# akio-tomiya/LatticeQCD.jl

Hardware: AMD Instinct MI355X
Metric: CG iters/sec (D^+D) & Dslash GFLOP/s, 32^3x64 SU(3) Wilson fp64 (higher is better)
Workload: dtype f64; 1 GPU; configs[3]: 32x32x32x64 Wilson D^+D CG (fixed-length window), fp64; dslash_variant=1, xcd_remap=2, xcd_nsub=16, xcd_ysplit=4, cg_fused=3, gauge_recon=12, gauge_recon_active=1, comm_backend=none, comm_requested=auto

## Files before the change

### latticeqcd.jl_amd/csrc/capi.hip

```cpp
#include "lqcd_internal.h"

#include <cstdio>
#include <cstdlib>
#include <cstring>
#include <mutex>

namespace lqcd {

static thread_local std::string g_err;
static std::mutex g_live_mu;
static std::vector<const lqcd_ctx_s*> g_live;
bool ctx_is_live(const lqcd_ctx_s* c) {
    std::lock_guard<std::mutex> lk(g_live_mu);
    for (const lqcd_ctx_s* p : g_live)
        if (p == c) return true;
    return false;
}
static void ctx_set_live(const lqcd_ctx_s* c, bool live) {
    std::lock_guard<std::mutex> lk(g_live_mu);
    for (size_t i = 0; i < g_live.size(); i++)
        if (g_live[i] == c) { g_live.erase(g_live.begin() + i); break; }
    if (live) g_live.push_back(c);
}
bool ctx_park_gauge(lqcd_gauge_s* g) {
    std::lock_guard<std::mutex> lk(g_live_mu);
    lqcd_ctx_s* c = g->ctx;
    bool live = false;
    for (const lqcd_ctx_s* p : g_live) live = live || p == c;
    if (!live || !c->tun.lazy_links || std::this_thread::get_id() == c->home_thread) return false;
    c->parked_gauges.push_back(g);
    return true;
}
int ctx_drain_parked(lqcd_ctx_s* c) {
    std::vector<lqcd_gauge_s*> mine;
    {
        std::lock_guard<std::mutex> lk(g_live_mu);
        mine.swap(c->parked_gauges);
    }
    for (lqcd_gauge_s* g : mine) (void)gauge_destroy_now(g);
    return LQCD_OK;
}
void set_error(const std::string& msg) { g_err = msg; }
int hip_fail(hipError_t e, const char* what, const char* file, int line) {
    g_err = std::string("HIP error: ") + hipGetErrorString(e) + " in " + what + " (" + file + ":" + std::to_string(line) + ")";
    (void)hipGetLastError();
    return LQCD_ERR_HIP;
}
int nccl_fail(ncclResult_t e, const char* what, const char* file, int line) {
    g_err = std::string("RCCL error: ") + ncclGetErrorString(e) + " in " + what + " (" + file + ":" + std::to_string(line) + ")";
    return LQCD_ERR_COMM;
}

lqcd_spinor_s* scratch_get(lqcd_ctx_s* c, int kind, int subset) {
    if (std::this_thread::get_id() == c->home_thread && !c->parked_gauges.empty()) (void)ctx_drain_parked(c);
    const int want_sub = subset == LQCD_FULL ? LQCD_FULL : LQCD_EVEN;
    for (lqcd_spinor_s* s : c->scratch)
        if (!s->in_use && s->kind == kind && (s->subset == LQCD_FULL) == (want_sub == LQCD_FULL)) {
            s->in_use = true;
            s->subset = subset;
            return s;
        }
    lqcd_spinor_s* s = nullptr;
    if (lqcd_spinor_create(c, &s, kind, subset) != LQCD_OK) return nullptr;
    s->in_use = true;
    c->scratch.push_back(s);
    return s;
}
void scratch_put(lqcd_spinor_s* s) {
    if (s) s->in_use = false;
}

int plaquette_local_sum(lqcd_gauge_s* g, const double2* const ghost[4], double* sum);
int gauge_pack_face(lqcd_gauge_s* g, int mu, double2* dst);

static int decompose(const int gL[4], const int pe[4], int rank, int L[4], int origin[4], int coord[4], int nf[4], int nb[4]) {
    int nranks = 1;
    for (int mu = 0; mu < 4; mu++) {
        ARGCHK(pe[mu] >= 1 && gL[mu] >= 2, "decompose: bad PE grid or lattice extent");
        ARGCHK(gL[mu] % pe[mu] == 0, "decompose: global extent not divisible by the PE grid");
        L[mu] = gL[mu] / pe[mu];
        ARGCHK(L[mu] % 2 == 0, "decompose: local extents must be even (checkerboard layout)");
        nranks *= pe[mu];
    }
    ARGCHK(rank >= 0 && rank < nranks, "decompose: rank outside the PE grid");
    int q = rank;
    for (int mu = 0; mu < 4; mu++) { coord[mu] = q % pe[mu]; q /= pe[mu]; origin[mu] = coord[mu] * L[mu]; }
    for (int mu = 0; mu < 4; mu++) {
        int cf[4] = {coord[0], coord[1], coord[2], coord[3]}, cb[4] = {coord[0], coord[1], coord[2], coord[3]};
        cf[mu] = (coord[mu] + 1) % pe[mu];
        cb[mu] = (coord[mu] + pe[mu] - 1) % pe[mu];
        nf[mu] = cf[0] + pe[0] * (cf[1] + pe[1] * (cf[2] + pe[2] * cf[3]));
        nb[mu] = cb[0] + pe[0] * (cb[1] + pe[1] * (cb[2] + pe[2] * cb[3]));
    }
    return LQCD_OK;
// ... 213 lines not shown
    if (!strcmp(key, "mixed_xfuse")) return &c->tun.mixed_xfuse;
    if (!strcmp(key, "mixed_defer_x")) return &c->tun.mixed_defer_x;
    if (!strcmp(key, "pair32_active")) return &c->tun.pair32_active;
    if (!strcmp(key, "stag_both")) return &c->tun.stag_both;
    if (!strcmp(key, "clover_fused")) return &c->tun.clover_fused;
    if (!strcmp(key, "clover_transport")) return &c->tun.clover_transport;
    if (!strcmp(key, "halo_stream_mode")) return &c->tun.halo_stream_mode;
    if (!strcmp(key, "cg_skip_done")) return &c->tun.cg_skip_done;
    if (!strcmp(key, "cg_small")) return &c->tun.cg_small;
    if (!strcmp(key, "cg_tgauge")) return &c->tun.cg_tgauge;
    if (!strcmp(key, "tgauge_active")) return &c->tun.tgauge_active;
    if (!strcmp(key, "cg_sweep_alt")) return &c->tun.cg_sweep_alt;
    if (!strcmp(key, "cg_sweep_alt_active")) return &c->tun.cg_sweep_alt_active;
    if (!strcmp(key, "dslash_sweep")) return &c->tun.dslash_sweep;
    if (!strcmp(key, "sweep_rev_active")) return &c->tun.sweep_rev_active;
    if (!strcmp(key, "dslash_xshare")) return &c->tun.dslash_xshare;
    if (!strcmp(key, "xshare_active")) return &c->tun.xshare_active;
    if (!strcmp(key, "dslash_yshare")) return &c->tun.dslash_yshare;
    if (!strcmp(key, "yshare_active")) return &c->tun.yshare_active;
    if (!strcmp(key, "nt_centre")) return &c->tun.nt_centre;
    if (!strcmp(key, "cg_persist")) return &c->tun.cg_persist;
    if (!strcmp(key, "md_remap")) return &c->tun.md_remap;
    if (!strcmp(key, "staple_recon")) return &c->tun.staple_recon;
    if (!strcmp(key, "staple_tile")) return &c->tun.staple_tile;
    if (!strcmp(key, "md_reunitarize")) return &c->tun.md_reunitarize;
    if (!strcmp(key, "nt_blas")) return &c->tun.nt_blas;
    if (!strcmp(key, "cg_fold_scalars")) return &c->tun.cg_fold_scalars;
    if (!strcmp(key, "halo_fuse")) return &c->tun.halo_fuse;
    if (!strcmp(key, "halo_fold")) return &c->tun.halo_fold;
    if (!strcmp(key, "halo_fold_active")) return &c->tun.halo_fold_active;
    if (!strcmp(key, "cg_defer_x")) return &c->tun.cg_defer_x;
    if (!strcmp(key, "cg_rring")) return &c->tun.cg_rring;
    if (!strcmp(key, "cg_rring_active")) return &c->tun.cg_rring_active;
    if (!strcmp(key, "staggered_parity_solve")) return &c->tun.staggered_parity_solve;
    if (!strcmp(key, "halo_tuned_us0")) return &c->tun.halo_tuned_us[0];
    if (!strcmp(key, "halo_tuned_us1")) return &c->tun.halo_tuned_us[1];
    if (!strcmp(key, "halo_tuned_us2")) return &c->tun.halo_tuned_us[2];
    if (!strcmp(key, "halo_tuned_us3")) return &c->tun.halo_tuned_us[3];
    if (!strcmp(key, "halo_tuned_us4")) return &c->tun.halo_tuned_us[4];
    if (!strcmp(key, "halo_inject_us")) return &c->tun.halo_inject_us;
    if (!strcmp(key, "halo_merge")) return &c->tun.halo_merge;
    if (!strcmp(key, "recon_active")) return &c->tun.recon_active;
    if (!strcmp(key, "variants_built")) return &c->tun.variants_built;
    if (!strcmp(key, "lds_pad_kb")) return &c->tun.lds_pad_kb;
    if (!strcmp(key, "xcd_nsub")) return &c->tun.xcd_nsub;
    if (!strcmp(key, "xcd_ysplit")) return &c->tun.xcd_ysplit;
#ifdef LQCD_ABLATE
    if (!strcmp(key, "dbg")) return &c->tun.dbg;
#endif
    if (!strcmp(key, "persist_per_cu")) return &c->tun.persist_per_cu;
    if (!strcmp(key, "dslash_pipe")) return &c->tun.dslash_pipe;
    if (!strcmp(key, "pipe_per_cu")) return &c->tun.pipe_per_cu;
    if (!strcmp(key, "pipe_grid")) return &c->tun.pipe_grid;
    if (!strcmp(key, "pipe_chunks_per_wg")) return &c->tun.pipe_chunks_per_wg;
    if (!strcmp(key, "pipe_min_chunks")) return &c->tun.pipe_min_chunks;
    if (!strcmp(key, "lazy_links")) return &c->tun.lazy_links;
    if (!strcmp(key, "lazy_merge")) return &c->tun.lazy_merge;
    if (!strcmp(key, "dw_batched")) return &c->tun.dw_batched;
    if (!strcmp(key, "dw_fused_cg")) return &c->tun.dw_fused_cg;
    if (!strcmp(key, "bicg_fused")) return &c->tun.bicg_fused;
    if (!strcmp(key, "gauge_delta")) return &c->tun.gauge_delta;
    if (!strcmp(key, "dslash_s18")) return &c->tun.dslash_s18;
    if (!strcmp(key, "bicg_mixed")) return &c->tun.bicg_mixed;
    if (!strcmp(key, "action_eo_solver")) return &c->tun.action_eo_solver;
    if (!strcmp(key, "bicg_xrp_active")) return &c->tun.bicg_xrp_active;
    if (!strcmp(key, "mrhs_active")) return &c->tun.mrhs_active;
    if (!strcmp(key, "meson_mrhs")) return &c->tun.meson_mrhs;
    if (!strcmp(key, "peer_timeout_ms")) return &c->peer.timeout_ms;
    return nullptr;
}
extern "C" int lqcd_ctx_set_param(lqcd_ctx_t c, const char* key, int value) {
    ARGCHK(c && key, "lqcd_ctx_set_param: null");
    if (!strcmp(key, "adopt_thread")) {
        {
            std::lock_guard<std::mutex> lk(g_live_mu);
            c->home_thread = std::this_thread::get_id();
        }
        return ctx_drain_parked(c);
    }
    int* p = param_ptr(c, key);
    ARGCHK(p, std::string("lqcd_ctx_set_param: unknown key ") + key);
    if (!strcmp(key, "dslash_block")) ARGCHK(value == 64 || value == 128 || value == 256, "dslash_block must be 64, 128 or 256");
    if (!strcmp(key, "halo_stream_mode")) ARGCHK(value >= -1 && value <= 4, "halo_stream_mode must be -1 (timed once) or 0..4");
    if (!strcmp(key, "cg_rring")) ARGCHK(value == 0 || value == 2 || value == 4 || value == 8, "cg_rring must be 0 (off), 2, 4 or 8 (it divides the 8 iterations of a captured burst)");
    if (!strcmp(key, "bicg_fused")) ARGCHK(value != 3, "bicg_fused must be 0, 1, 2 or 4 (3, the grid-barrier form, was measured slower and removed)");
    if (!strcmp(key, "halo_inject_us")) ARGCHK(value >= 0 && value <= 100000, "halo_inject_us: 0..100000");
    if ((!strcmp(key, "lazy_links") || !strcmp(key, "lazy_merge")) && !value) LQCHK(links_flush_of(c));
    if (*p != value) LQCHK(links_flush_of(c));
    *p = value;
    return LQCD_OK;
}
extern "C" int lqcd_ctx_get_param(lqcd_ctx_t c, const char* key, int* value) {
    ARGCHK(c && key && value, "lqcd_ctx_get_param: null");
    if (!strcmp(key, "dw_active")) { *value = c->tun.dw_active; return LQCD_OK; }
    if (!strcmp(key, "adopt_thread")) {
        std::lock_guard<std::mutex> lk(g_live_mu);
        *value = std::this_thread::get_id() == c->home_thread ? 1 : 0;
        return LQCD_OK;
    }
    if (!strcmp(key, "parked_fields")) {
        std::lock_guard<std::mutex> lk(g_live_mu);
        *value = (int)c->parked_gauges.size();
        return LQCD_OK;
    }
    if (!strcmp(key, "lazy_open")) { *value = c->lazy.kind; return LQCD_OK; }
    if (!strcmp(key, "lazy_deferred")) { *value = (int)c->lazy.done.size() + (c->lazy.has_pend ? 4 : 0) + (c->lazy.has_pp ? 4 : 0); return LQCD_OK; }
    int* p = param_ptr(c, key);
    ARGCHK(p, std::string("lqcd_ctx_get_param: unknown key ") + key);
    *value = *p;
    return LQCD_OK;
}

extern "C" int lqcd_comm_unique_id(unsigned char id[256]) {
    ARGCHK(id, "lqcd_comm_unique_id: null");
    static_assert(sizeof(ncclUniqueId) == 128, "ncclUniqueId is expected to be 128 bytes");
    for (int k = 0; k < 2; k++) {
        ncclUniqueId u;
        NCCLCHK(ncclGetUniqueId(&u));
        memcpy(id + 128 * k, &u, 128);
    }
    return LQCD_OK;
}
// ... 82 lines not shown
```

### latticeqcd.jl_amd/csrc/cg.hip

```cpp
#include "ops_internal.h"
#include "stencil_common.h"

#include <algorithm>
#include <cmath>

namespace lqcd {


__global__ void cg_scalar_alpha(double* s) {
    if (s[S_DONE] != 0.0) { s[S_XDONE] = 1.0; return; }
    s[S_ALPHA] = s[S_RR] / s[S_PQ];
}
__global__ void cg_scalar_beta(double* s) {
    if (s[S_DONE] != 0.0) return;
    const double rrn = s[S_RRNEW];
    s[S_BETA] = rrn / s[S_RR];
    s[S_RR] = rrn;
    s[S_ITERS] += 1.0;
    if (rrn < s[S_EPS]) s[S_DONE] = 1.0;
}

__global__ __launch_bounds__(UB) void cg_update_xr(const double* __restrict__ s, double2* __restrict__ x, double2* __restrict__ r,
                                                    const double2* __restrict__ p, const double2* __restrict__ q, size_t n,
                                                    double* partial) {
// ... 193 lines not shown
                double2 o;
                o.x = fma(be, pv.x, rv.x); o.y = fma(be, pv.y, rv.y);
                stx<NT>(pnext + i, o);
            }
        }
    } else {
        for (size_t i = (size_t)fb0 * UB + threadIdx.x; i < n; i += (size_t)nbf * UB) {
            const double2 pv = ldx<NT>(pk + i), rv = ldx<NT>(r + i);
            double2 o;
            o.x = fma(be, pv.x, rv.x); o.y = fma(be, pv.y, rv.y);
            stx<NT>(pnext + i, o);
        }
        if (fb0 == 0 && threadIdx.x == 0) s[S_AHIST + m] = al;
    }
    cg_beta_commit<FOLD>(s, fb, fb0 == 0);
}
__global__ __launch_bounds__(UB) void cg_flush_ring(const double* __restrict__ s, double2* __restrict__ x, CgRing ring, int m, size_t n) {
    if (s[S_DONE] != 0.0) return;
    double ah[8];
#pragma unroll
    for (int j = 0; j < 8; j++) ah[j] = j < m ? s[S_AHIST + j] : 0.0;
    for (size_t i = (size_t)blockIdx.x * UB + threadIdx.x; i < n; i += (size_t)gridDim.x * UB) {
        double2 xv = x[i];
#pragma unroll
        for (int j = 0; j < 8; j++) {
            if (j < m) {
                const double2 pj = ring.b[j][i];
                xv.x = fma(ah[j], pj.x, xv.x); xv.y = fma(ah[j], pj.y, xv.y);
            }
        }
        x[i] = xv;
    }
}
struct CgSlots { const double2* r[8]; };
template <bool NT>
__global__ __launch_bounds__(UB) void cg_batch_px(const double* __restrict__ s, double2* __restrict__ x, double2* __restrict__ p, CgSlots sl, int fin, size_t n) {
    const int np = (int)(s[S_ITERS] - s[S_BSTART]);
    if (np <= 0 || np > 8 || (!fin && s[S_DONE] != 0.0)) return;
    double al[8], be[8];
#pragma unroll
    for (int j = 0; j < 8; j++) { al[j] = j < np ? s[S_AHIST + j] : 0.0; be[j] = j < np ? s[S_BHIST + j] : 0.0; }
    for (size_t i = (size_t)blockIdx.x * UB + threadIdx.x; i < n; i += (size_t)gridDim.x * UB) {
        double2 xv = ldx<NT>(x + i), pv = ldx<NT>(p + i);
#pragma unroll
        for (int j = 0; j < 8; j++) {
            if (j < np) {
                xv.x = fma(al[j], pv.x, xv.x); xv.y = fma(al[j], pv.y, xv.y);
                if (!fin || j < np - 1) {
                    const double2 rv = ldx<NT>(sl.r[j] + i);
                    pv.x = fma(be[j], pv.x, rv.x); pv.y = fma(be[j], pv.y, rv.y);
                }
            }
        }
        stx<NT>(x + i, xv);
        if (!fin) stx<NT>(p + i, pv);
    }
}
__global__ __launch_bounds__(UB) void cg_update_p(const double* __restrict__ s, double2* __restrict__ p, const double2* __restrict__ r, size_t n) {
    if (s[S_DONE] != 0.0) return;
    const double be = s[S_BETA];
    for (size_t i = (size_t)blockIdx.x * UB + threadIdx.x; i < n; i += (size_t)gridDim.x * UB) {
        const double2 rv = r[i];
        double2 pv = p[i];
        pv.x = fma(be, pv.x, rv.x); pv.y = fma(be, pv.y, rv.y);
        p[i] = pv;
    }
}
__global__ __launch_bounds__(UB) void norm2_partial_kernel(const double2* __restrict__ a, size_t n, double* partial) {
    __shared__ double red[UB / 64];
    double acc = 0;
    for (size_t i = (size_t)blockIdx.x * UB + threadIdx.x; i < n; i += (size_t)gridDim.x * UB) {
        const double2 v = a[i];
        acc = fma(v.x, v.x, acc); acc = fma(v.y, v.y, acc);
    }
#pragma unroll
    for (int off = 32; off > 0; off >>= 1) acc += __shfl_down(acc, off, 64);
    if ((threadIdx.x & 63) == 0) red[threadIdx.x >> 6] = acc;
    __syncthreads();
// ... 55 lines not shown
static bool cg_small_ok(lqcd_op_s* op, int nbs) {
    lqcd_ctx_s* c = op->ctx;
    if (any_partitioned(c) || c->has_comm || nbs > 1024) return false;
    const int v = c->tun.dslash_variant;
#ifdef LQCD_VARIANTS
    if (op->kind == LQCD_WILSON && op->r == 1.0 && (v == 2 || v == 3)) return false;
#endif
    (void)v;
    if ((c->tun.dslash_pipe == 1 || c->tun.dslash_pipe == 3) && wilson_pipe_applies(c, op->kind, op->r, 2, op_fused_clover(op))) return false;
    return true;
}

int cg_work_get(lqcd_ctx_s* c, int kind, CgWork& w) {
    w.r = scratch_get(c, kind, LQCD_FULL); w.p = scratch_get(c, kind, LQCD_FULL);
    w.q = scratch_get(c, kind, LQCD_FULL); w.tmp = scratch_get(c, kind, LQCD_FULL);
    if (!(w.r && w.p && w.q && w.tmp)) { cg_work_put(w); return LQCD_ERR_HIP; }
    return LQCD_OK;
}
void cg_work_put(CgWork& w) {
    for (lqcd_spinor_s** f : {&w.r, &w.p, &w.q, &w.tmp}) { if (*f) scratch_put(*f); *f = nullptr; }
    for (lqcd_spinor_s*& f : w.more) { if (f) scratch_put(f); f = nullptr; }
}
static int cg_ring_wanted(lqcd_op_s* op) {
    const int k = op->ctx->tun.cg_defer_x;
    if (op->kind == LQCD_DOMAINWALL) return 2;
    if (k >= 3) return std::min(k, 8);
    return (k == 1 && any_partitioned(op->ctx)) ? 8 : 2;
}
static CgRing cg_ring_pending(const CgWork& w, int m) {
    CgRing ring;
    for (int j = 0; j < 8; j++) ring.b[j] = j < m ? w.buf((w.k - m + j) % w.ring)->data : nullptr;
    return ring;
}
static int cg_batch_launch(lqcd_ctx_s* c, lqcd_spinor_s* x, CgWork& w, int fin) {
    CgSlots sl;
    for (int j = 0; j < 8; j++) sl.r[j] = j < w.rring ? w.slot((j + 1) % w.rring)->data : nullptr;
    const dim3 g(stream_grid(c, x->elems)), b(UB);
    if (c->tun.nt_blas) hipLaunchKernelGGL(cg_batch_px<true>, g, b, 0, c->stream, c->d_scal, x->data, w.p->data, sl, fin, x->elems);
    else hipLaunchKernelGGL(cg_batch_px<false>, g, b, 0, c->stream, c->d_scal, x->data, w.p->data, sl, fin, x->elems);
    HIPCHK(hipGetLastError());
    return LQCD_OK;
}
int cg_flush_x(lqcd_op_s* op, lqcd_spinor_s* x, CgWork& w) {
    lqcd_ctx_s* c = op->ctx;
    if (w.form == CgForm::RRing) {
        if (w.flushed || w.k == 0) return LQCD_OK;
        w.flushed = true;
        return cg_batch_launch(c, x, w, 1);
    }
    const bool deferred = w.form == CgForm::DeferX;
    if (deferred && w.ring > 2) {
        const int m = w.k % w.ring;
        if (m == 0) return LQCD_OK;
        hipLaunchKernelGGL(cg_flush_ring, dim3(stream_grid(c, x->elems)), dim3(UB), 0, c->stream, c->d_scal, x->data, cg_ring_pending(w, m), m, x->elems);
        HIPCHK(hipGetLastError());
        w.k += w.ring - m;
        return LQCD_OK;
    }
    if (!deferred || !(w.k & 1)) return LQCD_OK;
    const size_t n = x->elems;
    hipLaunchKernelGGL(cg_flush_kernel, dim3(stream_grid(c, n)), dim3(UB), 0, c->stream, c->d_scal, x->data, w.p->data, n);
    HIPCHK(hipGetLastError());
    w.k++;
    return LQCD_OK;
}

int cg_finish(lqcd_op_s* op, lqcd_spinor_s* x, CgWork& w, bool flush) {
    int st = flush ? cg_flush_x(op, x, w) : LQCD_OK;
    if (w.tgauge) {
        const int sr = spinor_gauge_rotate(op->ctx, w.gfix, x->data, x->data, 1);
        if (st == LQCD_OK) st = sr;
        w.tgauge = false;
// ... 186 lines not shown
        }
    }
    const CgUpd u = {dim3(nbu + npack), x->data, pk->data, po->data, n, nbu, h, npx};
    if (!defer) hipLaunchKernelGGL(cg_update_xp, u.grid, dim3(UB), 0, c->stream, c->d_scal, x->data, w.p->data, w.r->data, n);
    else switch ((c->tun.nt_blas ? 4 : 0) | (fold ? 2 : 0) | (fp ? 1 : 0)) {
        case 0: cg_launch_update_defer<false, false, false>(c, w, u); break;
        case 1: cg_launch_update_defer<false, false, true>(c, w, u); break;
        case 2: cg_launch_update_defer<false, true, false>(c, w, u); break;
        case 3: cg_launch_update_defer<false, true, true>(c, w, u); break;
        case 4: cg_launch_update_defer<true, false, false>(c, w, u); break;
        case 5: cg_launch_update_defer<true, false, true>(c, w, u); break;
        case 6: cg_launch_update_defer<true, true, false>(c, w, u); break;
        default: cg_launch_update_defer<true, true, true>(c, w, u); break;
    }
    w.p_packed = fp;
    if (fp) w.pack_epoch = ++c->halo_epoch;
    HIPCHK(hipGetLastError());
    w.k++;
    return LQCD_OK;
}

int cg_enqueue_iteration(lqcd_op_s* op, lqcd_spinor_s* x, CgWork& w) {
    switch (w.form) {
        case CgForm::Reference: case CgForm::NormFused: return cg_iter_reference(op, x, w);
        case CgForm::Fused: case CgForm::DeferX: return cg_iter_fused(op, x, w);
        case CgForm::Small: return cg_iter_small(op, x, w);
        case CgForm::RRing: return cg_enqueue_rring(op, x, w);
        case CgForm::Unset: break;
    }
    set_error("CG: the work vectors were never set up (cg_setup fixes the iteration form)");
    return LQCD_ERR_ARG;
}

static bool cg_more_get(lqcd_ctx_s* c, CgWork& w, int K) {
    bool ok = K >= 2;
    for (int j = 0; j < K - 2 && ok; j++) {
        if (!w.more[j]) w.more[j] = scratch_get(c, w.r->kind, LQCD_FULL);
        ok = w.more[j] != nullptr;
    }
    if (!ok) for (lqcd_spinor_s*& f : w.more) { if (f) scratch_put(f); f = nullptr; }
    return ok;
}
static CgForm cg_choose_form(lqcd_op_s* op, CgWork& w) {
    lqcd_ctx_s* c = op->ctx;
    const int fused = c->tun.cg_fused;
    if (fused >= 2 && c->tun.cg_small && cg_small_ok(op, stencil_num_partials(c, op->kind, op->r, 2, 0, op_fused_clover(op)))) return CgForm::Small;
    if (cg_more_get(c, w, cg_rring_wanted(op, w))) return CgForm::RRing;
    if (fused >= 2 && c->tun.cg_defer_x) return CgForm::DeferX;
    return fused >= 2 ? CgForm::Fused : fused ? CgForm::NormFused : CgForm::Reference;
}

int cg_setup(lqcd_op_s* op, lqcd_spinor_s* x, lqcd_spinor_s* b, CgWork& w, double eps, double* rr0) {
    lqcd_ctx_s* c = op->ctx;
    const size_t n = x->elems;
    LQCHK(halo_schedule_settle(op));
    w.tgauge = cg_tgauge_wanted(op);
    c->tun.tgauge_active = w.tgauge ? 1 : 0;
    w.links_t = w.tgauge ? op->gauge->data12t : nullptr;
    w.gfix = w.tgauge ? op->gauge->gfix : nullptr;
    w.gauge_version = op->gauge->version;
    if (w.tgauge) LQCHK(spinor_gauge_rotate(c, w.gfix, x->data, x->data, 0));
    LQCHK(op_apply_async(op, w.tmp, x, 0, nullptr, nullptr, w.links_t));
    LQCHK(op_apply_async(op, w.q, w.tmp, 1, nullptr, nullptr, w.links_t));
    if (w.tgauge) LQCHK(spinor_gauge_rotate(c, w.gfix, w.r->data, b->data, 0));
    else HIPCHK(hipMemcpyAsync(w.r->data, b->data, n * sizeof(double2), hipMemcpyDeviceToDevice, c->stream));
    LQCHK(blas_axpy(c, -1.0, 0.0, w.q->data, w.r->data, n));
    HIPCHK(hipMemcpyAsync(w.p->data, w.r->data, n * sizeof(double2), hipMemcpyDeviceToDevice, c->stream));
    LQCHK(blas_norm2(c, w.r->data, n, rr0, true));
    double init[12] = {*rr0, 0, 0, 0, 0, 0, eps, 0, 0, 0, 0, 0};
    static_assert(S_BSTART - S_RR == 11, "cg_setup: the scalar block it initialises ends at S_BSTART");
    HIPCHK(hipMemcpyAsync(c->d_scal + S_RR, init, sizeof(init), hipMemcpyHostToDevice, c->stream));
    HIPCHK(hipStreamSynchronize(c->stream));
    w.k = 0; w.p_packed = false; w.flushed = false;
    w.form = cg_choose_form(op, w);
    w.rring = w.form == CgForm::RRing ? c->tun.cg_rring : 0;
    c->tun.cg_rring_active = w.rring;
    w.sweep_alt = c->tun.cg_sweep_alt != 0 && w.tgauge && (w.form == CgForm::RRing || w.form == CgForm::Fused || w.form == CgForm::DeferX);
    c->tun.cg_sweep_alt_active = w.sweep_alt ? 1 : 0;
    w.ring = 2;
    if (w.form == CgForm::DeferX) {
        int want = cg_ring_wanted(op);
        if (c->tun.graph != 0 && !any_partitioned(c) && (8 % want) != 0) want = 2;
        if (cg_more_get(c, w, want)) w.ring = want;
    }
    return LQCD_OK;
}

int cg_run(lqcd_op_s* op, lqcd_spinor_s* x, lqcd_spinor_s* b, double eps, int maxiter, bool fixed, int* iters, double* final_rr) {
    lqcd_ctx_s* c = op->ctx;
    HIPCHK(hipSetDevice(c->device));
    CgWork w;
    int st = cg_work_get(c, x->kind, w);
    double rr = 0;
    int it = 0;
    bool converged = false;
    bool one_launch = st == LQCD_OK && maxiter > 0 && c->tun.graph == 0 && cg_persist_ok(op);
    if (one_launch) {
        bool gave_up = false;
        st = cg_persist_run(op, x, b, w, fixed ? -1.0 : eps, maxiter, &it, &rr, &converged, &gave_up);
        if (gave_up) { one_launch = false; it = 0; rr = 0; converged = false; c->tun.cg_persist = 0; }
        else if (st == LQCD_OK && !std::isfinite(rr)) { set_error("CG: residual is not finite"); st = LQCD_ERR_NOT_CONVERGED; }
    }
    if (st == LQCD_OK && !one_launch) st = cg_setup(op, x, b, w, fixed ? -1.0 : eps, &rr);
    if (st == LQCD_OK && !one_launch && !fixed && rr < eps) converged = true;
    const int check_every = 8;
    const bool adaptive = !fixed && c->tun.graph == 0 && w.form == CgForm::Small;
    int next_burst = check_every, it_prev = 0;
    double rr_prev = rr;
    const bool use_graph = c->tun.graph != 0 && !any_partitioned(c) && !(c->has_comm && c->peer.on);
    hipGraph_t graph = nullptr;
    hipGraphExec_t gexec = nullptr;
    while (st == LQCD_OK && !one_launch && !converged && it < maxiter) {
        int burst = std::min(adaptive ? next_burst : check_every, maxiter - it);
        if (fixed && !use_graph) burst = maxiter - it;
        if (use_graph && burst == check_every) {
            if (!gexec) {
                if (c->tun.halo_stream_mode < 0) c->tun.halo_stream_mode = 0;
                hipError_t ge = hipStreamBeginCapture(c->stream, hipStreamCaptureModeThreadLocal);
                if (ge != hipSuccess) { st = hip_fail(ge, "hipStreamBeginCapture", __FILE__, __LINE__); break; }
                for (int k = 0; k < burst && st == LQCD_OK; k++) st = cg_enqueue_iteration(op, x, w);
                ge = hipStreamEndCapture(c->stream, &graph);
                if (st == LQCD_OK && ge != hipSuccess) st = hip_fail(ge, "hipStreamEndCapture", __FILE__, __LINE__);
                if (st == LQCD_OK) {
                    ge = hipGraphInstantiate(&gexec, graph, nullptr, nullptr, 0);
                    if (ge != hipSuccess) st = hip_fail(ge, "hipGraphInstantiate", __FILE__, __LINE__);
                }
                if (st != LQCD_OK) break;
            }
            hipError_t ge = hipGraphLaunch(gexec, c->stream);
            if (ge != hipSuccess) { st = hip_fail(ge, "hipGraphLaunch", __FILE__, __LINE__); break; }
        } else {
            for (int k = 0; k < burst && st == LQCD_OK; k++) st = cg_enqueue_iteration(op, x, w);
        }
        if (st != LQCD_OK) break;
        if (fixed && use_graph && it + burst < maxiter) { it += burst; continue; }
        hipError_t e = hipMemcpyAsync(c->h_scal, c->d_scal + S_RR, 8 * sizeof(double), hipMemcpyDeviceToHost, c->stream);
        if (e == hipSuccess) e = hipStreamSynchronize(c->stream);
        if (e != hipSuccess) { st = hip_fail(e, "cg scalar readback", __FILE__, __LINE__); break; }
        rr = c->h_scal[S_RR - S_RR];
        it = (int)c->h_scal[S_ITERS - S_RR];
        if (c->h_scal[S_DONE - S_RR] != 0.0) converged = true;
        if (!std::isfinite(rr)) { set_error("CG: residual is not finite"); st = LQCD_ERR_NOT_CONVERGED; }
// ... 117 lines not shown
```

### latticeqcd.jl_amd/csrc/lqcd_internal.h

```cpp
#pragma once
#include <hip/hip_runtime.h>
#include <rccl/rccl.h>
#include <stdint.h>
#include <mutex>
#include <string>
#include <thread>
#include <vector>

#include "../../include/lqcd_hip.h"

namespace lqcd {

#ifdef LQCD_F32
typedef float real;
typedef float2 real2;
#define LQCD_PNS p32
inline namespace p32 {}
namespace p64 {}
#else
typedef double real;
typedef double2 real2;
#define LQCD_PNS p64
inline namespace p64 {}
namespace p32 {}
// ... 217 lines not shown
    int i = cls;
    for (; i + 15 * FB < nblocks; i += 16 * FB) {
        double t[16];
#pragma unroll
        for (int k = 0; k < 16; k++) t[k] = partial[(size_t)(i + k * FB) * si];
#pragma unroll
        for (int q = 0; q < 4; q++) { s0 += t[4 * q]; s1 += t[4 * q + 1]; s2 += t[4 * q + 2]; s3 += t[4 * q + 3]; }
    }
    for (; i + 7 * FB < nblocks; i += 8 * FB) {
        double t[8];
#pragma unroll
        for (int k = 0; k < 8; k++) t[k] = partial[(size_t)(i + k * FB) * si];
#pragma unroll
        for (int q = 0; q < 2; q++) { s0 += t[4 * q]; s1 += t[4 * q + 1]; s2 += t[4 * q + 2]; s3 += t[4 * q + 3]; }
    }
    for (; i + 3 * FB < nblocks; i += 4 * FB) {
        s0 += partial[(size_t)i * si];
        s1 += partial[(size_t)(i + FB) * si];
        s2 += partial[(size_t)(i + 2 * FB) * si];
        s3 += partial[(size_t)(i + 3 * FB) * si];
    }
    for (; i < nblocks; i += FB) s0 += partial[(size_t)i * si];
    return (s0 + s1) + (s2 + s3);
}
__device__ inline double shfl_tree_sum(double s) {
#pragma unroll
    for (int off = 32; off > 0; off >>= 1) s += __shfl_down(s, off, 64);
    return s;
}

enum { S_RED0 = 0, S_RR = 8, S_PQ = 9, S_ALPHA = 10, S_BETA = 11, S_DONE = 12, S_ITERS = 13, S_EPS = 14, S_RRNEW = 15, S_XDONE = 16, S_RROLD = 17, S_APREV = 18,
       S_BSTART = 19,
       S_AHIST = 64,
       S_BHIST = 72 };
enum { B_RHO = 24, B_R0V = 26, B_VV = 28, B_ALPHA = 29, B_SS = 31, B_TS = 32, B_TT = 34, B_OMEGA = 35, B_RR = 37, B_RHO1 = 38, B_BETA = 40,
       B_DONE = 42, B_ITERS = 43, B_EPS = 44, B_HALF = 45, B_RES = 46, B_RHOB = 47, B_TS5 = 49, B_UNSURE = 54, B_XDONE = 55, B_END = 56 };
__device__ inline void cg_scalar_step(double* s, int op) {
    if (op == 1) {
        if (s[S_DONE] != 0.0) { s[S_XDONE] = 1.0; return; }
        s[S_ALPHA] = s[S_RR] / s[S_PQ];
    } else if (op == 2) {
        if (s[S_DONE] != 0.0) return;
        const double rrn = s[S_RRNEW];
        s[S_BETA] = rrn / s[S_RR];
        s[S_RR] = rrn;
        s[S_ITERS] += 1.0;
        if (rrn < s[S_EPS]) s[S_DONE] = 1.0;
    } else if (op == 7 || op == 9) {
        if (s[S_DONE] != 0.0) { s[S_XDONE] = 1.0; return; }
        if (op == 9) s[S_BSTART] = s[S_ITERS];
        const double al = s[S_RR] / s[S_PQ];
        s[S_ALPHA] = al;
        s[S_AHIST + ((int)(s[S_ITERS] - s[S_BSTART]) & 7)] = al;
    } else if (op == 8) {
        if (s[S_DONE] != 0.0) return;
        const double rrn = s[S_RRNEW];
        const double be = rrn / s[S_RR];
        s[S_BETA] = be;
        s[S_BHIST + ((int)(s[S_ITERS] - s[S_BSTART]) & 7)] = be;
        s[S_RR] = rrn;
        s[S_ITERS] += 1.0;
        if (rrn < s[S_EPS]) s[S_DONE] = 1.0;
    } else if (op >= 3 && op <= 6) {
        if (s[B_DONE] != 0.0) return;
        if (op == 3) {
            c2 rho = {s[B_RHO], s[B_RHO + 1]}, r0v = {s[B_R0V], s[B_R0V + 1]};
            const c2 a = bicg_alpha(rho, r0v);
            s[B_ALPHA] = a.re;
            s[B_ALPHA + 1] = a.im;
        } else if (op == 4) {
            s[B_HALF] = (s[B_SS] < s[B_EPS]) ? 1.0 : 0.0;
        } else if (op == 5) {
            c2 ts = {s[B_TS], s[B_TS + 1]};
            const c2 w = bicg_omega(ts, s[B_TT], s[B_HALF] != 0.0);
            s[B_OMEGA] = w.re;
            s[B_OMEGA + 1] = w.im;
        } else {
            s[B_ITERS] += 1.0;
            const double rr = (s[B_HALF] != 0.0) ? s[B_SS] : s[B_RR];
            s[B_RES] = rr;
            if (s[B_HALF] != 0.0 || rr < s[B_EPS]) { s[B_DONE] = 1.0; return; }
            if (!(fabs(rr) <= 1.79e308)) { s[B_DONE] = 2.0; return; }
            c2 rho1 = {s[B_RHO1], s[B_RHO1 + 1]}, rho = {s[B_RHO], s[B_RHO + 1]}, al = {s[B_ALPHA], s[B_ALPHA + 1]}, om = {s[B_OMEGA], s[B_OMEGA + 1]};
            const c2 b = bicg_beta(rho1, rho, al, om);
            s[B_BETA] = b.re;
            s[B_BETA + 1] = b.im;
            s[B_RHO] = rho1.re; s[B_RHO + 1] = rho1.im;
        }
    }
}

__host__ __device__ inline uint64_t splitmix64(uint64_t x) {
// ... 43 lines not shown
        int j = b >> 3;
        p = j & 1; j >>= 1;
        const int per_pass = m.cpr * m.LT;
        const int pass = fdiv(j, m.d_perpass);
        j -= pass * per_pass;
        const int t = fdiv(j, m.d_cpr), mm = j - t * m.cpr, sd = xcd + 8 * pass;
        int s;
        if (m.ysplit > 1) {
            const int sz = fdiv(sd, m.d_ysplit), sy = sd - sz * m.ysplit;
            const int zz = fdiv(mm, m.d_ty), yy = mm - zz * m.ty;
            s = (sz * m.tz + zz) * m.cpp + sy * m.ty + yy;
        } else {
            s = sd * m.cpr + mm;
        }
        chunk = t * m.cps + s;
        return;
    }
    int lb = b;
    if (m.remap && !(m.nblocks & 7)) lb = (b & 7) * (m.nblocks >> 3) + (b >> 3);
    chunk = lb >> 1; p = lb & 1;
}

struct Ctx;

struct Tunables {
    int dslash_block = 128;
    int xcd_remap = 2;
    int dslash_variant = 1;
    int nt_gauge = 1;
    int nt_store = 1;
    int cg_fused = 3;
    int cg_rring = 8;
    int cg_rring_active = 0;
    int graph = 0;
    int persist_per_cu = 2;
    int dslash_pipe = 2;
    int pipe_per_cu = 0;
    int pipe_chunks_per_wg = 2;
    int pipe_grid = 0;
    int pipe_min_chunks = 8;
#ifdef LQCD_ABLATE
    int dbg = 0;
#endif
    int xcd_ysplit = 4;
    int xcd_nsub = 16;
    int lds_pad_kb = 0;
    int halo_merge = 1;
    int clover_fused = 1;
    int halo_stream_mode = -1;
    int halo_tuned_us[5] = {0, 0, 0, 0, 0};
    int halo_inject_us = 0;
    int staggered_parity_solve = 1;
    int halo_fold = 1;
    int halo_fold_active = 0;
    int halo_fuse = 2;
    int cg_fold_scalars = 1;
    int nt_blas = 1;
    int md_reunitarize = 1;
    int staple_recon = 1;
    int staple_tile = 1;
    int md_remap = 1;
    int cg_defer_x = 1;
    int cg_persist = 1;
    int cg_small = 1;
    int cg_tgauge = 1;
    int tgauge_active = 0;
// ... 300 lines not shown
    lqcd_spinor_s* view_of = nullptr;
    int nviews = 0;
    bool zombie = false;
};

struct lqcd_op_s {
    lqcd_ctx_s* ctx;
    int kind;
    lqcd_gauge_s* gauge;
    double km;
    double r;
    int bc[4];
    double csw = 0.0;
    double2* clover = nullptr;
    uint64_t clover_version = 0;
    lqcd_spinor_s* clover_tmp = nullptr;
    double2* clover_inv = nullptr;
    uint64_t clover_inv_version = 0;
    double2* clover_lambda = nullptr;
    int bicg32_hint[2][4] = {};
    int bicg_mrhs_hint = 0;
    int bicg_hint = 0;
    int L5 = 0;
    double dw_M = 0.0;
    lqcd_op_s* dw_wilson = nullptr;
    lqcd_spinor_s* dw_work[8] = {};
    double* dw_partial = nullptr;
    size_t dw_partial_n = 0;
};

namespace lqcd {

constexpr int MAX_PARTIAL_BLOCKS = 4096;
constexpr int SCAL_DOUBLES = 96;

void set_error(const std::string& msg);
int hip_fail(hipError_t e, const char* what, const char* file, int line);
int nccl_fail(ncclResult_t e, const char* what, const char* file, int line);

#define HIPCHK(x)                                                              \
    do {                                                                       \
        hipError_t _e = (x);                                                   \
        if (_e != hipSuccess) return lqcd::hip_fail(_e, #x, __FILE__, __LINE__); \
    } while (0)
#define NCCLCHK(x)                                                              \
    do {                                                                        \
        ncclResult_t _e = (x);                                                  \
        if (_e != ncclSuccess) return lqcd::nccl_fail(_e, #x, __FILE__, __LINE__); \
    } while (0)
#define LQCHK(x)                       \
    do {                               \
        int _s = (x);                  \
        if (_s != LQCD_OK) return _s;  \
    } while (0)
#define ARGCHK(cond, msg)                     \
    do {                                      \
        if (!(cond)) {                        \
            lqcd::set_error(msg);             \
            return LQCD_ERR_ARG;              \
        }                                     \
    } while (0)


struct CommXfer {
    const void* send;
    void* recv;
    size_t bytes;
// ... 156 lines not shown
```

### latticeqcd.jl_amd/csrc/ops_internal.h

```cpp
#pragma once
#include "lqcd_internal.h"

#include <functional>
#include <vector>

namespace lqcd {

double2* spinor_block(lqcd_spinor_s* s, int p);
int stream_grid(lqcd_ctx_s* c, size_t n);

StencilCall make_hop_call(lqcd_op_s* op, lqcd_spinor_s* out, lqcd_spinor_s* in, lqcd_spinor_s* xin, double a, double b, int dagger);
int check_full(lqcd_op_s* op, lqcd_spinor_s* a, lqcd_spinor_s* b, const char* who);
int make_full_call(lqcd_op_s* op, lqcd_spinor_s* out, lqcd_spinor_s* in, int dagger, StencilCall& s);
void apply_bc(lqcd_ctx_s* c, const int bc[4]);
void split_general_r(const StencilCall& s, StencilCall& s1, StencilCall& s2);

constexpr int UB = 256;
enum class CgForm { Unset, Reference, NormFused, Fused, DeferX, Small, RRing };
struct CgWork {
    lqcd_spinor_s *r, *p, *q, *tmp;
    uint64_t pack_epoch = 0;
    bool p_packed = false;
    CgForm form = CgForm::Unset;
    int k = 0;
    int ring = 2;
    lqcd_spinor_s* more[6] = {nullptr, nullptr, nullptr, nullptr, nullptr, nullptr};
    lqcd_spinor_s* buf(int j) const { return j == 0 ? p : j == 1 ? q : more[j - 2]; }
    int rring = 0;
    bool flushed = false;
    lqcd_spinor_s* slot(int j) const { return j == 0 ? r : j == 1 ? q : more[j - 2]; }
    bool tgauge = false;
    const double2* links_t = nullptr;
    const double2* gfix = nullptr;
    uint64_t gauge_version = 0;
    bool sweep_alt = false;
};
int cg_work_get(lqcd_ctx_s* c, int kind, CgWork& w);
void cg_work_put(CgWork& w);
int cg_enqueue_iteration(lqcd_op_s* op, lqcd_spinor_s* x, CgWork& w);
int cg_flush_x(lqcd_op_s* op, lqcd_spinor_s* x, CgWork& w);
int cg_setup(lqcd_op_s* op, lqcd_spinor_s* x, lqcd_spinor_s* b, CgWork& w, double eps, double* rr0);
int cg_finish(lqcd_op_s* op, lqcd_spinor_s* x, CgWork& w, bool flush = true);
bool cg_gauge_moved(lqcd_op_s* op, const CgWork& w);
bool cg_persist_ok(lqcd_op_s* op);
int cg_persist_run(lqcd_op_s* op, lqcd_spinor_s* x, lqcd_spinor_s* b, CgWork& w, double eps, int maxiter, int* iters, double* rr, bool* converged, bool* gave_up);
typedef std::function<int(double2* out, const double2* in)> ApplyFn;
int cg_generic(lqcd_ctx_s* c, const ApplyFn& A, size_t n, double2* x, const double2* b, double2* r, double2* p, double2* q, double eps,
               int maxiter, int* iters, double* final_rr);
int cg_launch_update_xp(lqcd_ctx_s* c, double2* x, double2* p, const double2* r, size_t n);

int bicgstab_core(lqcd_ctx_s* c, const ApplyFn& A, size_t n, double2* x, const double2* b, double2* const w[6], double eps, int maxiter, int* iters, double* final_rr);

int ms_zeta_launch(lqcd_ctx_s* c, double* d_ms, int ns, int stop_when_frozen);

#ifdef __HIPCC__
typedef double v2dd __attribute__((ext_vector_type(2)));
template <bool NT> __device__ inline double2 ldx(const double2* p) {
    if constexpr (NT) { v2dd v = __builtin_nontemporal_load(reinterpret_cast<const v2dd*>(p)); double2 r; r.x = v.x; r.y = v.y; return r; }
    else return *p;
}
template <bool NT> __device__ inline void stx(double2* p, double2 v) {
// ... 101 lines not shown
```

Baseline: 1212 iter/s.

## Deepen CG residual ring to batch up to 32 deferred x/p updates

Measured after the change: 1243 iter/s, median of 6. 1.03x the previous value.

```diff
diff --git a/latticeqcd.jl_amd/csrc/capi.hip b/latticeqcd.jl_amd/csrc/capi.hip
--- a/latticeqcd.jl_amd/csrc/capi.hip
+++ b/latticeqcd.jl_amd/csrc/capi.hip
@@ -1,5 +1,6 @@
 #include "lqcd_internal.h"
 
+#include <algorithm>
 #include <cstdio>
 #include <cstdlib>
 #include <cstring>
@@ -60,6 +61,7 @@
             s->subset = subset;
             return s;
         }
+    if (c->tun.scratch_max > 0 && (int)c->scratch.size() >= c->tun.scratch_max) { set_error("scratch pool: all scratch_max work fields are in use"); return nullptr; }
     lqcd_spinor_s* s = nullptr;
     if (lqcd_spinor_create(c, &s, kind, subset) != LQCD_OK) return nullptr;
     s->in_use = true;
@@ -339,6 +341,9 @@
     if (!strcmp(key, "cg_defer_x")) return &c->tun.cg_defer_x;
     if (!strcmp(key, "cg_rring")) return &c->tun.cg_rring;
     if (!strcmp(key, "cg_rring_active")) return &c->tun.cg_rring_active;
+    if (!strcmp(key, "cg_rring_mult")) return &c->tun.cg_rring_mult;
+    if (!strcmp(key, "cg_rring_depth_active")) return &c->tun.cg_rring_depth_active;
+    if (!strcmp(key, "scratch_max")) return &c->tun.scratch_max;
     if (!strcmp(key, "staggered_parity_solve")) return &c->tun.staggered_parity_solve;
     if (!strcmp(key, "halo_tuned_us0")) return &c->tun.halo_tuned_us[0];
     if (!strcmp(key, "halo_tuned_us1")) return &c->tun.halo_tuned_us[1];
@@ -390,11 +395,14 @@
     if (!strcmp(key, "dslash_block")) ARGCHK(value == 64 || value == 128 || value == 256, "dslash_block must be 64, 128 or 256");
     if (!strcmp(key, "halo_stream_mode")) ARGCHK(value >= -1 && value <= 4, "halo_stream_mode must be -1 (timed once) or 0..4");
     if (!strcmp(key, "cg_rring")) ARGCHK(value == 0 || value == 2 || value == 4 || value == 8, "cg_rring must be 0 (off), 2, 4 or 8 (it divides the 8 iterations of a captured burst)");
+    if (!strcmp(key, "cg_rring_mult")) ARGCHK((value == 1 || value == 2 || value == 4) && std::max(c->tun.cg_rring, 1) * value <= RRING_MAX, "cg_rring_mult must be 1, 2 or 4 with cg_rring x cg_rring_mult <= 32");
+    if (!strcmp(key, "scratch_max")) ARGCHK(value >= 0, "scratch_max: 0 (no limit) or the number of work fields the scratch pool may hold");
     if (!strcmp(key, "bicg_fused")) ARGCHK(value != 3, "bicg_fused must be 0, 1, 2 or 4 (3, the grid-barrier form, was measured slower and removed)");
     if (!strcmp(key, "halo_inject_us")) ARGCHK(value >= 0 && value <= 100000, "halo_inject_us: 0..100000");
     if ((!strcmp(key, "lazy_links") || !strcmp(key, "lazy_merge")) && !value) LQCHK(links_flush_of(c));
     if (*p != value) LQCHK(links_flush_of(c));
     *p = value;
+    if (!strcmp(key, "cg_rring_mult")) c->tun.cg_rring_mult_set = 1;
     return LQCD_OK;
 }
 extern "C" int lqcd_ctx_get_param(lqcd_ctx_t c, const char* key, int* value) {
diff --git a/latticeqcd.jl_amd/csrc/cg.hip b/latticeqcd.jl_amd/csrc/cg.hip
--- a/latticeqcd.jl_amd/csrc/cg.hip
+++ b/latticeqcd.jl_amd/csrc/cg.hip
@@ -249,18 +249,34 @@
         x[i] = xv;
     }
 }
-struct CgSlots { const double2* r[8]; };
-template <bool NT>
+struct CgSlots { const double2* r[RRING_MAX]; };
+template <bool NT, int DEPTH>
 __global__ __launch_bounds__(UB) void cg_batch_px(const double* __restrict__ s, double2* __restrict__ x, double2* __restrict__ p, CgSlots sl, int fin, size_t n) {
     const int np = (int)(s[S_ITERS] - s[S_BSTART]);
-    if (np <= 0 || np > 8 || (!fin && s[S_DONE] != 0.0)) return;
-    double al[8], be[8];
-#pragma unroll
-    for (int j = 0; j < 8; j++) { al[j] = j < np ? s[S_AHIST + j] : 0.0; be[j] = j < np ? s[S_BHIST + j] : 0.0; }
+    if (np <= 0 || np > DEPTH || (!fin && s[S_DONE] != 0.0)) return;
+    double al[DEPTH], be[DEPTH];
+#pragma unroll
+    for (int j = 0; j < DEPTH; j++) { al[j] = j < np ? s[S_AHIST + j] : 0.0; be[j] = j < np ? s[S_BHIST + j] : 0.0; }
+    if (DEPTH >= 32 && !fin && np == DEPTH) {
+        for (size_t i = (size_t)blockIdx.x * UB + threadIdx.x; i < n; i += (size_t)gridDim.x * UB) {
+            double2 xv = ldx<NT>(x + i), pv = ldx<NT>(p + i);
+            double2 rv[DEPTH];
+#pragma unroll
+            for (int j = 0; j < DEPTH; j++) rv[j] = ldx<NT>(sl.r[j] + i);
+#pragma unroll
+            for (int j = 0; j < DEPTH; j++) {
+                xv.x = fma(al[j], pv.x, xv.x); xv.y = fma(al[j], pv.y, xv.y);
+                pv.x = fma(be[j], pv.x, rv[j].x); pv.y = fma(be[j], pv.y, rv[j].y);
+            }
+            stx<NT>(x + i, xv);
+            stx<NT>(p + i, pv);
+        }
+        return;
+    }
     for (size_t i = (size_t)blockIdx.x * UB + threadIdx.x; i < n; i += (size_t)gridDim.x * UB) {
         double2 xv = ldx<NT>(x + i), pv = ldx<NT>(p + i);
 #pragma unroll
-        for (int j = 0; j < 8; j++) {
+        for (int j = 0; j < DEPTH; j++) {
             if (j < np) {
                 xv.x = fma(al[j], pv.x, xv.x); xv.y = fma(al[j], pv.y, xv.y);
                 if (!fin || j < np - 1) {
@@ -382,12 +398,19 @@
     for (int j = 0; j < 8; j++) ring.b[j] = j < m ? w.buf((w.k - m + j) % w.ring)->data : nullptr;
     return ring;
 }
+template <int DEPTH>
+static void cg_batch_launch_depth(lqcd_ctx_s* c, bool nt, dim3 g, dim3 b, lqcd_spinor_s* x, CgWork& w, const CgSlots& sl, int fin) {
+    if (nt) hipLaunchKernelGGL((cg_batch_px<true, DEPTH>), g, b, 0, c->stream, c->d_scal, x->data, w.p->data, sl, fin, x->elems);
+    else hipLaunchKernelGGL((cg_batch_px<false, DEPTH>), g, b, 0, c->stream, c->d_scal, x->data, w.p->data, sl, fin, x->elems);
+}
 static int cg_batch_launch(lqcd_ctx_s* c, lqcd_spinor_s* x, CgWork& w, int fin) {
     CgSlots sl;
-    for (int j = 0; j < 8; j++) sl.r[j] = j < w.rring ? w.slot((j + 1) % w.rring)->data : nullptr;
+    for (int j = 0; j < RRING_MAX; j++) sl.r[j] = j < w.rring ? w.slot((j + 1) % w.rring)->data : nullptr;
     const dim3 g(stream_grid(c, x->elems)), b(UB);
-    if (c->tun.nt_blas) hipLaunchKernelGGL(cg_batch_px<true>, g, b, 0, c->stream, c->d_scal, x->data, w.p->data, sl, fin, x->elems);
-    else hipLaunchKernelGGL(cg_batch_px<false>, g, b, 0, c->stream, c->d_scal, x->data, w.p->data, sl, fin, x->elems);
+    const bool nt = c->tun.nt_blas != 0;
+    if (w.rring <= 8) cg_batch_launch_depth<8>(c, nt, g, b, x, w, sl, fin);
+    else if (w.rring == 16) cg_batch_launch_depth<16>(c, nt, g, b, x, w, sl, fin);
+    else cg_batch_launch_depth<32>(c, nt, g, b, x, w, sl, fin);
     HIPCHK(hipGetLastError());
     return LQCD_OK;
 }
@@ -640,6 +663,13 @@
     return LQCD_ERR_ARG;
 }
 
+static int cg_rring_mult_wanted(lqcd_op_s* op, int K) {
+    lqcd_ctx_s* c = op->ctx;
+    int M = c->tun.cg_rring_mult;
+    if (!c->tun.cg_rring_mult_set && stencil_num_partials(c, op->kind, op->r, 2, 0, op_fused_clover(op)) <= 1024) M = 1;
+    while (M > 1 && K * M > RRING_MAX) M >>= 1;
+    return M;
+}
 static bool cg_more_get(lqcd_ctx_s* c, CgWork& w, int K) {
     bool ok = K >= 2;
     for (int j = 0; j < K - 2 && ok; j++) {
@@ -653,7 +683,10 @@
     lqcd_ctx_s* c = op->ctx;
     const int fused = c->tun.cg_fused;
     if (fused >= 2 && c->tun.cg_small && cg_small_ok(op, stencil_num_partials(c, op->kind, op->r, 2, 0, op_fused_clover(op)))) return CgForm::Small;
-    if (cg_more_get(c, w, cg_rring_wanted(op, w))) return CgForm::RRing;
+    if (const int K = cg_rring_wanted(op, w)) {
+        for (int M = cg_rring_mult_wanted(op, K); M >= 1; M >>= 1)
+            if (cg_more_get(c, w, K * M)) { w.rring = K * M; w.rring_k = K; return CgForm::RRing; }
+    }
     if (fused >= 2 && c->tun.cg_defer_x) return CgForm::DeferX;
     return fused >= 2 ? CgForm::Fused : fused ? CgForm::NormFused : CgForm::Reference;
 }
@@ -680,9 +713,10 @@
     HIPCHK(hipMemcpyAsync(c->d_scal + S_RR, init, sizeof(init), hipMemcpyHostToDevice, c->stream));
     HIPCHK(hipStreamSynchronize(c->stream));
     w.k = 0; w.p_packed = false; w.flushed = false;
+    w.rring = w.rring_k = 0;
     w.form = cg_choose_form(op, w);
-    w.rring = w.form == CgForm::RRing ? c->tun.cg_rring : 0;
-    c->tun.cg_rring_active = w.rring;
+    c->tun.cg_rring_active = w.rring_k;
+    c->tun.cg_rring_depth_active = w.rring;
     w.sweep_alt = c->tun.cg_sweep_alt != 0 && w.tgauge && (w.form == CgForm::RRing || w.form == CgForm::Fused || w.form == CgForm::DeferX);
     c->tun.cg_sweep_alt_active = w.sweep_alt ? 1 : 0;
     w.ring = 2;
@@ -711,11 +745,12 @@
     }
     if (st == LQCD_OK && !one_launch) st = cg_setup(op, x, b, w, fixed ? -1.0 : eps, &rr);
     if (st == LQCD_OK && !one_launch && !fixed && rr < eps) converged = true;
-    const int check_every = 8;
+    int check_every = 8;
     const bool adaptive = !fixed && c->tun.graph == 0 && w.form == CgForm::Small;
     int next_burst = check_every, it_prev = 0;
     double rr_prev = rr;
     const bool use_graph = c->tun.graph != 0 && !any_partitioned(c) && !(c->has_comm && c->peer.on);
+    if (use_graph && w.form == CgForm::RRing && w.rring > 0) check_every = (check_every + w.rring - 1) / w.rring * w.rring;
     hipGraph_t graph = nullptr;
     hipGraphExec_t gexec = nullptr;
     while (st == LQCD_OK && !one_launch && !converged && it < maxiter) {
diff --git a/latticeqcd.jl_amd/csrc/lqcd_internal.h b/latticeqcd.jl_amd/csrc/lqcd_internal.h
--- a/latticeqcd.jl_amd/csrc/lqcd_internal.h
+++ b/latticeqcd.jl_amd/csrc/lqcd_internal.h
@@ -273,7 +273,10 @@
 enum { S_RED0 = 0, S_RR = 8, S_PQ = 9, S_ALPHA = 10, S_BETA = 11, S_DONE = 12, S_ITERS = 13, S_EPS = 14, S_RRNEW = 15, S_XDONE = 16, S_RROLD = 17, S_APREV = 18,
        S_BSTART = 19,
        S_AHIST = 64,
-       S_BHIST = 72 };
+       S_BHIST = 96,
+       S_HIST_END = 128 };
+constexpr int RRING_MAX = 32;
+static_assert(S_BHIST - S_AHIST == RRING_MAX && S_HIST_END - S_BHIST == RRING_MAX && (RRING_MAX & (RRING_MAX - 1)) == 0, "the CG histories hold RRING_MAX entries each");
 enum { B_RHO = 24, B_R0V = 26, B_VV = 28, B_ALPHA = 29, B_SS = 31, B_TS = 32, B_TT = 34, B_OMEGA = 35, B_RR = 37, B_RHO1 = 38, B_BETA = 40,
        B_DONE = 42, B_ITERS = 43, B_EPS = 44, B_HALF = 45, B_RES = 46, B_RHOB = 47, B_TS5 = 49, B_UNSURE = 54, B_XDONE = 55, B_END = 56 };
 __device__ inline void cg_scalar_step(double* s, int op) {
@@ -292,13 +295,13 @@
         if (op == 9) s[S_BSTART] = s[S_ITERS];
         const double al = s[S_RR] / s[S_PQ];
         s[S_ALPHA] = al;
-        s[S_AHIST + ((int)(s[S_ITERS] - s[S_BSTART]) & 7)] = al;
+        s[S_AHIST + ((int)(s[S_ITERS] - s[S_BSTART]) & (RRING_MAX - 1))] = al;
     } else if (op == 8) {
         if (s[S_DONE] != 0.0) return;
         const double rrn = s[S_RRNEW];
         const double be = rrn / s[S_RR];
         s[S_BETA] = be;
-        s[S_BHIST + ((int)(s[S_ITERS] - s[S_BSTART]) & 7)] = be;
+        s[S_BHIST + ((int)(s[S_ITERS] - s[S_BSTART]) & (RRING_MAX - 1))] = be;
         s[S_RR] = rrn;
         s[S_ITERS] += 1.0;
         if (rrn < s[S_EPS]) s[S_DONE] = 1.0;
@@ -408,6 +411,10 @@
     int cg_fused = 3;
     int cg_rring = 8;
     int cg_rring_active = 0;
+    int cg_rring_mult = 4;
+    int scratch_max = 0;
+    int cg_rring_mult_set = 0;
+    int cg_rring_depth_active = 0;
     int graph = 0;
     int persist_per_cu = 2;
     int dslash_pipe = 2;
@@ -774,7 +781,8 @@
 namespace lqcd {
 
 constexpr int MAX_PARTIAL_BLOCKS = 4096;
-constexpr int SCAL_DOUBLES = 96;
+constexpr int SCAL_DOUBLES = 144;
+static_assert(S_HIST_END + 9 <= SCAL_DOUBLES, "d_scal: the CG histories must end below the staging doubles");
 
 void set_error(const std::string& msg);
 int hip_fail(hipError_t e, const char* what, const char* file, int line);
diff --git a/latticeqcd.jl_amd/csrc/ops_internal.h b/latticeqcd.jl_amd/csrc/ops_internal.h
--- a/latticeqcd.jl_amd/csrc/ops_internal.h
+++ b/latticeqcd.jl_amd/csrc/ops_internal.h
@@ -24,9 +24,10 @@
     CgForm form = CgForm::Unset;
     int k = 0;
     int ring = 2;
-    lqcd_spinor_s* more[6] = {nullptr, nullptr, nullptr, nullptr, nullptr, nullptr};
+    lqcd_spinor_s* more[RRING_MAX - 2] = {};
     lqcd_spinor_s* buf(int j) const { return j == 0 ? p : j == 1 ? q : more[j - 2]; }
     int rring = 0;
+    int rring_k = 0;
     bool flushed = false;
     lqcd_spinor_s* slot(int j) const { return j == 0 ? r : j == 1 ? q : more[j - 2]; }
     bool tgauge = false;
```
